# snarkify/sirius

Measured on AMD Instinct MI355X. Metric: IVC fold-steps/s (CycleFold IVC::next hot path, Poseidon-shaped synthetic trace, 2^k rows), higher is better.
Workload: dtype u256 (modular; 9 x 29-bit / 8 x 32-bit limbs)

## Files before the change

sirius_amd/csrc/msm.h:

```cpp
#pragma once
#include "curve.cuh"
#include "devrt.h"
#include "glv.cuh"
#include "stripes.h"
#include "tuning.h"

#include <cstdlib>

namespace srs {
namespace msm {

constexpr int WBITS = 16;
constexpr int NWIN = 16;
constexpr int NWIN_COMPACT = 8;
constexpr uint32_t PAY_ENDO = 1u << 30;
constexpr uint32_t NBUCKET = 1u << (WBITS - 1);

constexpr uint32_t SORT_THREADS = 1024;
constexpr uint32_t SORT_TILE_MIN = 8192;
constexpr uint32_t SORT_TARGET_BLOCKS = 256;
constexpr uint32_t SEG = 128, SEG_BUCKETS = NBUCKET / SEG;
constexpr uint32_t SORT_TILE2 = 8192;
constexpr uint64_t TWO_PASS_MIN_SLOTS = 1ull << 23;
constexpr uint32_t PLAN_THREADS = 1024;
constexpr uint32_t ACC_THREADS = 256;
constexpr uint32_t ACC_L0_LOG = 4, ACC_L0 = 1u << ACC_L0_LOG;
constexpr uint32_t ACC_L1_LOG = 3, ACC_L1 = 1u << ACC_L1_LOG;
constexpr uint32_t FINAL_THREADS = 256;
constexpr uint32_t FINAL_FANIN = 512;
constexpr int MAX_LEVELS = 8;
constexpr uint32_t RED_ROWS = 256;
constexpr uint32_t RED_COLS = NBUCKET / RED_ROWS;
constexpr uint32_t RED_THREADS = 4 * RED_COLS;
constexpr uint32_t ACC1_QUAD_MAX = 1u << 17;
constexpr uint32_t BATCH_ARGS = 16;
constexpr uint32_t LANDING_SLOTS = 16;
constexpr uint32_t NORM_G = 16;
constexpr uint32_t SLOT_LOG = 6;
constexpr uint32_t SLOT_L0_MIN_LOG = 2, SLOT_L0_MAX_LOG = 16;
constexpr int WBITS_W = 20;
constexpr int NWIN_W = 13;
constexpr uint32_t NSEG_W = 16;
// ... 63 lines not shown
```

sirius_amd/csrc/msm.hip:

```cpp
#define SRS_F29_CHAIN 1
#include "msm.h"
#include "tuning.h"
#include "curve29.cuh"
#include "prof.h"

#include <algorithm>
#include <cstdlib>
#include <numeric>
#include <vector>

namespace srs {
namespace msm {

__device__ __forceinline__ uint32_t upper_bucket(const uint32_t *__restrict__ tp, uint32_t t) {
    uint32_t lo = 0, hi = NBUCKET;
    while (hi - lo > 1) {
        uint32_t mid = (lo + hi) >> 1;
        if (tp[mid] <= t) lo = mid; else hi = mid;
    }
    return lo;
}

template <class C>
__global__ void k_table_step(const affine_t *__restrict__ prev, xyzz_t *__restrict__ tmp, uint32_t n, int nbits) {
// ... 88 lines not shown
    gen.x = F::one();
    if (C::ID == 0) {
        gen.y = F::dbl(F::one());
    } else {
        fe_t y;
        const uint32_t yc[8] = {0x823f272cu, 0x833fc48du, 0xf1181294u, 0x2d270d45u, 0x06a45d63u, 0xcf135e75u, 0x00000002u, 0u};
        for (int j = 0; j < 8; ++j) y.v[j] = yc[j];
        gen.y = F::to_mont(y);
    }
    tmp[i] = Ec<C>::mul_canon(k, gen);
}

template <class C>
__global__ void k_on_curve(const affine_t *__restrict__ pts, uint32_t n, uint32_t *__restrict__ bad) {
    uint32_t i = blockIdx.x * blockDim.x + threadIdx.x;
    if (i >= n) return;
    if (!Ec<C>::is_on_curve(table_unform<C>(pts[i]))) atomicAdd(bad, 1u);
}

struct BatchDesc {
    const fe_t *ptr[BATCH_ARGS];
    uint32_t n[BATCH_ARGS];
    uint32_t base[BATCH_ARGS];
};

__device__ __forceinline__ void recode_half(const uint32_t (&k)[4], bool neg, uint16_t *__restrict__ d, size_t n) {
    const uint32_t top = neg ? 0x7FFFu : 0x8000u;
    uint32_t carry = 0;
#pragma unroll
    for (int w = 0; w < NWIN_COMPACT; ++w) {
        const uint32_t v = ((k[w >> 1] >> ((w & 1) * 16)) & 0xFFFFu) + carry;
        const bool borrow = v > top;
        const uint32_t mag = borrow ? 0x10000u - v : v;
        const bool minus = borrow != neg;
        carry = borrow ? 1u : 0u;
        d[(size_t)w * n] = (uint16_t)(mag ? ((mag - 1u) | (minus ? 0x8000u : 0u)) : 0xFFFFu);
    }
}

template <class C, bool COMPACT>
__global__ void k_digits(BatchDesc bd, uint16_t *__restrict__ dig, size_t dig_stride, int is_mont, uint32_t rank, uint32_t world,
                         uint32_t *__restrict__ count_zero, uint32_t n_zero) {
    using S = typename C::S;
    uint32_t m = blockIdx.y;
    uint32_t n = bd.n[m];
    uint32_t i = blockIdx.x * blockDim.x + threadIdx.x;
    for (uint32_t j = (blockIdx.y * gridDim.x + blockIdx.x) * blockDim.x + threadIdx.x; j < n_zero; j += gridDim.x * gridDim.y * blockDim.x)
        count_zero[j] = 0;
    if (i >= n) return;
    fe_t s = bd.ptr[m][Stripes{rank, world}.global_index((size_t)i)];
    if (is_mont) s = S::from_mont(s);
    uint16_t *d = dig + (size_t)m * dig_stride;
    if (COMPACT) {
        const glv_t g = glv_decompose<C>(s);
        recode_half(g.k1, g.neg1, d + i, n);
        recode_half(g.k2, g.neg2, d + (size_t)NWIN_COMPACT * n + i, n);
        return;
    }
    uint32_t carry = 0;
#pragma unroll
    for (int w = 0; w < NWIN; ++w) {
        uint32_t raw = (s.v[w >> 1] >> ((w & 1) * 16)) & 0xFFFFu;
        uint32_t v = raw + carry;
        uint32_t code;
        if (v > 0x8000u) {
            code = ((0x10000u - v) - 1u) | 0x8000u;
            carry = 1;
        } else {
            code = v ? (v - 1u) : 0xFFFFu;
            carry = 0;
        }
        d[(size_t)w * n + i] = (uint16_t)code;
    }
}

template <class Fn>
__device__ __forceinline__ void for_each_digit(const uint16_t *__restrict__ d, uint32_t lo, uint32_t hi, Fn fn) {
    uint32_t head = lo;
    while (head < hi && (reinterpret_cast<uintptr_t>(d + head) & 15u)) ++head;
    for (uint32_t i = lo + threadIdx.x; i < head; i += blockDim.x) fn(i, (uint32_t)d[i]);
    const uint32_t nvec = (hi - head) / 8;
    const uint4 *v = reinterpret_cast<const uint4 *>(d + head);
    auto eight = [&](uint32_t q, const uint4 &x) {
        const uint32_t i0 = head + q * 8;
        fn(i0 + 0, x.x & 0xFFFFu); fn(i0 + 1, x.x >> 16);
        fn(i0 + 2, x.y & 0xFFFFu); fn(i0 + 3, x.y >> 16);
        fn(i0 + 4, x.z & 0xFFFFu); fn(i0 + 5, x.z >> 16);
        fn(i0 + 6, x.w & 0xFFFFu); fn(i0 + 7, x.w >> 16);
    };
    uint32_t q = threadIdx.x;
    for (; q + 3 * blockDim.x < nvec; q += 4 * blockDim.x) {
        const uint4 x0 = v[q], x1 = v[q + blockDim.x], x2 = v[q + 2 * blockDim.x], x3 = v[q + 3 * blockDim.x];
        eight(q, x0); eight(q + blockDim.x, x1); eight(q + 2 * blockDim.x, x2); eight(q + 3 * blockDim.x, x3);
    }
    for (; q < nvec; q += blockDim.x) eight(q, v[q]);
    for (uint32_t i = head + nvec * 8 + threadIdx.x; i < hi; i += blockDim.x) fn(i, (uint32_t)d[i]);
}

__device__ __forceinline__ void tile_histogram(uint32_t *h, const uint16_t *__restrict__ d, uint32_t lo, uint32_t hi) {
    for (uint32_t b = threadIdx.x; b < NBUCKET; b += blockDim.x) h[b] = 0;
    __syncthreads();
    for_each_digit(d, lo, hi, [&](uint32_t, uint32_t code) {
        if (code != 0xFFFFu) atomicAdd(&h[code & 0x7FFFu], 1u);
    });
    __syncthreads();
}

__global__ void SRS_KERNEL_BOUNDS(SORT_THREADS, 1)
    k_hist(const uint16_t *__restrict__ dig, size_t dig_stride, BatchDesc bd,
           uint32_t *__restrict__ count , uint32_t SORT_TILE,
           uint32_t *__restrict__ tile_hist ) {
    __shared__ uint32_t h[NBUCKET];
    uint32_t m = blockIdx.z, w = blockIdx.y;
    uint32_t n = bd.n[m];
    uint32_t lo = blockIdx.x * SORT_TILE;
    const uint32_t T1 = gridDim.x * NWIN, t1 = w * gridDim.x + blockIdx.x;
    if (lo >= n) {
        if (tile_hist)
            for (uint32_t sgm = threadIdx.x; sgm < SEG; sgm += blockDim.x) tile_hist[((size_t)m * SEG + sgm) * T1 + t1] = 0;
        return;
    }
    uint32_t hi = lo + SORT_TILE < n ? lo + SORT_TILE : n;
    const uint16_t *d = dig + (size_t)m * dig_stride + (size_t)w * n;
    tile_histogram(h, d, lo, hi);
    uint32_t *cnt = count + (size_t)m * NBUCKET;
    const uint32_t rot = ((blockIdx.y * gridDim.x + blockIdx.x) * 128u) & (NBUCKET - 1);
    for (uint32_t i = threadIdx.x; i < NBUCKET; i += blockDim.x) {
        const uint32_t b = (i + rot) & (NBUCKET - 1);
        uint32_t c = h[b];
        if (c) atomicAdd(&cnt[b], c);
    }
    if (tile_hist) {
        for (uint32_t sgm = threadIdx.x; sgm < SEG; sgm += blockDim.x) {
            uint32_t c = 0;
            for (uint32_t b = 0; b < SEG_BUCKETS; ++b) c += h[sgm * SEG_BUCKETS + ((b + sgm) & (SEG_BUCKETS - 1))];
            tile_hist[((size_t)m * SEG + sgm) * T1 + t1] = c;
        }
    }
}

__device__ __forceinline__ uint32_t block_exclusive_scan(uint32_t v, uint32_t *lds, uint32_t *total);

__global__ void SRS_KERNEL_BOUNDS(1024, 1)
    k_scan_seg(uint32_t *__restrict__ tile_hist, uint32_t T1, const uint32_t *__restrict__ plan, size_t plan_stride) {
    __shared__ uint32_t lds[64];
    const uint32_t sgm = blockIdx.x, m = blockIdx.y;
    uint32_t *row = tile_hist + ((size_t)m * SEG + sgm) * T1;
    const uint32_t base = plan[(size_t)m * plan_stride + (size_t)sgm * SEG_BUCKETS];
    uint32_t carry = 0;
    for (uint32_t at = 0; at < T1; at += blockDim.x) {
        const uint32_t i = at + threadIdx.x;
        const uint32_t v = i < T1 ? row[i] : 0;
        uint32_t total;
        const uint32_t ex = block_exclusive_scan(v, lds, &total);
        if (i < T1) row[i] = base + carry + ex;
        carry += total;
    }
}

constexpr uint32_t GRP_PER = 16, GRP_SUB = SORT_THREADS * GRP_PER;
template <bool COMPACT>
__device__ __forceinline__ uint32_t payload_base(uint32_t w, uint32_t table_stride, uint32_t base) {
    if (COMPACT) return ((w & (NWIN_COMPACT - 1)) * table_stride + base) | (w >= NWIN_COMPACT ? PAY_ENDO : 0u);
    return w * table_stride + base;
}
template <bool COMPACT>
__global__ void SRS_KERNEL_BOUNDS(SORT_THREADS, 1)
    k_group(const uint16_t *__restrict__ dig, size_t dig_stride, BatchDesc bd, const uint32_t *__restrict__ tile_hist,
            uint16_t *__restrict__ gkey, uint32_t *__restrict__ gpay, size_t g_stride, uint32_t table_stride, uint32_t SORT_TILE,
            const uint32_t *__restrict__ plan, size_t plan_stride, uint16_t *__restrict__ tb, size_t tb_stride, uint32_t arr) {
    __shared__ uint32_t cur[SEG], cnt[SEG], lb[SEG], sc[64];
    __shared__ uint32_t spay[GRP_SUB];
    __shared__ uint16_t skey[GRP_SUB];
    const uint32_t m = blockIdx.z, w = blockIdx.y, tid = threadIdx.x;
    if (tb) {
        const uint32_t *tp = plan + (size_t)m * plan_stride + (size_t)arr * (NBUCKET + 1);
        uint16_t *map = tb + (size_t)m * tb_stride;
        const uint32_t waves = gridDim.x * gridDim.y * (blockDim.x >> 6);
        const uint32_t wv = (blockIdx.y * gridDim.x + blockIdx.x) * (blockDim.x >> 6) + (tid >> 6), lane = tid & 63u;
        for (uint32_t b = wv; b < NBUCKET; b += waves) {
            const uint32_t s = tp[b], e = tp[b + 1];
            for (uint32_t t = s + lane; t < e; t += 64) map[t] = (uint16_t)b;
        }
    }
    const uint32_t n = bd.n[m];
    const uint32_t lo = blockIdx.x * SORT_TILE;
    if (lo >= n) return;
    const uint32_t hi = lo + SORT_TILE < n ? lo + SORT_TILE : n;
    const uint32_t T1 = gridDim.x * NWIN, t1 = w * gridDim.x + blockIdx.x;
    for (uint32_t sgm = tid; sgm < SEG; sgm += blockDim.x) cur[sgm] = tile_hist[((size_t)m * SEG + sgm) * T1 + t1];
    const uint16_t *d = dig + (size_t)m * dig_stride + (size_t)w * n;
    uint16_t *ok = gkey + (size_t)m * g_stride;
    uint32_t *op = gpay + (size_t)m * g_stride;
    const uint32_t pay0 = payload_base<COMPACT>(w, table_stride, bd.base[m]);
    for (uint32_t sub = lo; sub < hi; sub += GRP_SUB) {
        for (uint32_t sgm = tid; sgm < SEG; sgm += blockDim.x) cnt[sgm] = 0;
        __syncthreads();
        const uint32_t i0 = sub + tid * GRP_PER;
        uint32_t code[GRP_PER], rank[GRP_PER];
        if (i0 + GRP_PER <= hi && (reinterpret_cast<uintptr_t>(d + i0) & 15u) == 0) {
            const uint4 *v = reinterpret_cast<const uint4 *>(d + i0);
#pragma unroll
            for (uint32_t q = 0; q < GRP_PER / 8; ++q) {
                const uint4 x = v[q];
                code[8 * q + 0] = x.x & 0xFFFFu; code[8 * q + 1] = x.x >> 16;
                code[8 * q + 2] = x.y & 0xFFFFu; code[8 * q + 3] = x.y >> 16;
                code[8 * q + 4] = x.z & 0xFFFFu; code[8 * q + 5] = x.z >> 16;
                code[8 * q + 6] = x.w & 0xFFFFu; code[8 * q + 7] = x.w >> 16;
            }
        } else {
#pragma unroll
            for (uint32_t k = 0; k < GRP_PER; ++k) code[k] = i0 + k < hi ? (uint32_t)d[i0 + k] : 0xFFFFu;
        }
#pragma unroll
        for (uint32_t k = 0; k < GRP_PER; ++k)
            rank[k] = code[k] != 0xFFFFu ? atomicAdd(&cnt[(code[k] & 0x7FFFu) / SEG_BUCKETS], 1u) : 0u;
        __syncthreads();
        uint32_t n_sub;
        const uint32_t ex = block_exclusive_scan(tid < SEG ? cnt[tid] : 0u, sc, &n_sub);
        if (tid < SEG) lb[tid] = ex;
        __syncthreads();
#pragma unroll
        for (uint32_t k = 0; k < GRP_PER; ++k) {
            if (code[k] != 0xFFFFu) {
                const uint32_t bkt = code[k] & 0x7FFFu, pos = lb[bkt / SEG_BUCKETS] + rank[k];
                skey[pos] = (uint16_t)bkt;
                spay[pos] = (pay0 + i0 + k) | ((code[k] & 0x8000u) << 16);
            }
        }
        __syncthreads();
        for (uint32_t i = tid; i < n_sub; i += blockDim.x) {
            const uint32_t key = skey[i], sgm = key / SEG_BUCKETS, g = cur[sgm] + (i - lb[sgm]);
            ok[g] = (uint16_t)key;
            op[g] = spay[i];
        }
        __syncthreads();
        if (tid < SEG) cur[tid] += cnt[tid];
    }
}

constexpr uint32_t S2_PER = 8, S2_RANGE = 2 * SEG_BUCKETS;
static_assert(SORT_TILE2 == SORT_THREADS * S2_PER, "k_scatter2: one tile = S2_PER entries per thread");
__global__ void SRS_KERNEL_BOUNDS(SORT_THREADS, 2)
    k_scatter2(const uint16_t *__restrict__ gkey, const uint32_t *__restrict__ gpay, size_t g_stride,
               const uint32_t *__restrict__ plan, size_t plan_stride, uint32_t *__restrict__ cursor ,
               uint32_t *__restrict__ sorted, size_t sorted_stride, uint32_t TILE2) {
    __shared__ uint32_t cnt[S2_RANGE], lb[S2_RANGE], gb[S2_RANGE], sc[64];
    __shared__ uint32_t spay[SORT_TILE2];
    __shared__ uint16_t skey[SORT_TILE2];
    const uint32_t m = blockIdx.y, tid = threadIdx.x;
    const uint32_t total = plan[(size_t)m * plan_stride + NBUCKET];
    const uint32_t n_tiles = (total + TILE2 - 1) / TILE2, per_xcd = (n_tiles + 7) / 8;
    if (blockIdx.x / 8 >= per_xcd) return;
    const uint32_t tile_id = (blockIdx.x % 8) * per_xcd + blockIdx.x / 8;
    if (tile_id >= n_tiles) return;
    const uint32_t lo = tile_id * TILE2;
    if (lo >= total) return;
    const uint32_t hi = lo + TILE2 < total ? lo + TILE2 : total;
    const uint16_t *key = gkey + (size_t)m * g_stride;
    const uint32_t *pay = gpay + (size_t)m * g_stride;
// ... 31 lines not shown
    if (tid < S2_RANGE) {
        lb[tid] = ex;
        gb[tid] = c ? atomicAdd(&cur[b_lo + tid], c) : 0u;
    }
    __syncthreads();
#pragma unroll
    for (uint32_t k = 0; k < S2_PER; ++k) {
        if (kk[k] != 0xFFFFu) {
            const uint32_t pos = lb[kk[k] - b_lo] + rank[k];
            skey[pos] = (uint16_t)(kk[k] - b_lo);
            spay[pos] = pp[k];
        }
    }
    __syncthreads();
    for (uint32_t i = tid; i < n_tile; i += blockDim.x) {
        const uint32_t b = skey[i];
        out[gb[b] + (i - lb[b])] = spay[i];
    }
}

#ifndef SCATTER_RES_INFLIGHT
#define SCATTER_RES_INFLIGHT 4
#endif
template <bool COMPACT>
__global__ void SRS_KERNEL_BOUNDS(SORT_THREADS, 1)
    k_scatter(const uint16_t *__restrict__ dig, size_t dig_stride, BatchDesc bd,
              uint32_t *__restrict__ cursor , uint32_t *__restrict__ sorted,
              size_t sorted_stride, uint32_t table_stride, uint32_t SORT_TILE) {
    __shared__ uint32_t h[NBUCKET];
    uint32_t m = blockIdx.z, w = blockIdx.y;
    uint32_t n = bd.n[m];
    uint32_t lo = blockIdx.x * SORT_TILE;
    if (lo >= n) return;
    uint32_t hi = lo + SORT_TILE < n ? lo + SORT_TILE : n;
    const uint16_t *d = dig + (size_t)m * dig_stride + (size_t)w * n;
    tile_histogram(h, d, lo, hi);
    uint32_t *cur = cursor + (size_t)m * NBUCKET;
    constexpr int RES = SCATTER_RES_INFLIGHT;
    for (uint32_t b0 = threadIdx.x; b0 < NBUCKET; b0 += RES * blockDim.x) {
        uint32_t c[RES], r[RES];
#pragma unroll
        for (int u = 0; u < RES; ++u) c[u] = b0 + u * blockDim.x < NBUCKET ? h[b0 + u * blockDim.x] : 0u;
#pragma unroll
        for (int u = 0; u < RES; ++u) r[u] = c[u] ? atomicAdd(&cur[b0 + u * blockDim.x], c[u]) : 0u;
#pragma unroll
        for (int u = 0; u < RES; ++u) if (c[u]) h[b0 + u * blockDim.x] = r[u];
    }
    __syncthreads();
    uint32_t *out = sorted + (size_t)m * sorted_stride;
    const uint32_t pay0 = payload_base<COMPACT>(w, table_stride, bd.base[m]);
    for_each_digit(d, lo, hi, [&](uint32_t i, uint32_t code) {
        if (code != 0xFFFFu) {
            uint32_t pos = atomicAdd(&h[code & 0x7FFFu], 1u);
            out[pos] = (pay0 + i) | ((code & 0x8000u) << 16);
        }
    });
}

struct Link {
    uint32_t base[MAX_LEVELS + 1][NSEG_W + 1];
};
__device__ __forceinline__ uint32_t link_segment(const uint32_t *__restrict__ base, uint32_t t) {
    uint32_t v = 0;
#pragma unroll
    for (uint32_t u = 1; u < NSEG_W; ++u) v += (t >= base[u]) ? 1u : 0u;
    return v;
}

struct WideDesc {
    const fe_t *ptr;
    uint32_t n, base;
    uint32_t rank, world;
    int is_mont;
};

template <class C>
__device__ __forceinline__ void wide_codes(const WideDesc &wd, uint32_t i, uint32_t (&code)[NWIN_W]) {
// ... 1159 lines not shown
    return (lg >= 2 && lg <= 8) ? (uint32_t)lg : SLOT_LOG;
}
static uint32_t slot_want_cap() { return 4u; }

struct LevelShape {
    uint64_t M;
    int levels;
    size_t plan_stride;
    uint64_t cap0, cap1;
    uint32_t quad_max;
};
struct SetShape : LevelShape {
    bool two_pass;
    uint32_t tile, tiles;
};
struct NarrowShape : SetShape { uint32_t l0_log; };
struct SlotShape : SetShape { uint32_t S, nred; };
struct WideShape : LevelShape { uint32_t l0_log, T, tiles_g; };

static void sort_shape(SetShape &h, uint32_t n_max, uint32_t batch) {
    h.M = (uint64_t)n_max * NWIN;
    h.quad_max = acc1_quad_max();
    h.two_pass = use_two_pass(h.M, batch);
    h.tile = (uint32_t)((h.M * batch + SORT_TARGET_BLOCKS - 1) / SORT_TARGET_BLOCKS);
    h.tile = (h.tile + 1023u) & ~1023u;
    if (h.tile < SORT_TILE_MIN) h.tile = SORT_TILE_MIN;
    h.tiles = ceil_div(n_max, h.tile);
}
static NarrowShape narrow_shape(uint32_t n_max, uint32_t batch) {
    NarrowShape h;
    sort_shape(h, n_max, batch);
    h.l0_log = l0_log_for(h.M);
    h.levels = levels_for((h.M + (1ull << h.l0_log) - 1) >> h.l0_log);
    h.plan_stride = (size_t)(h.levels + 1) * (NBUCKET + 1) + 4;
    h.cap0 = (h.M >> h.l0_log) + NBUCKET + 1;
    h.cap1 = h.cap0 / ACC_L1 + NBUCKET + 1;
    return h;
}
static SlotShape slot_shape(uint32_t n_max, uint32_t batch) {
    SlotShape h;
    sort_shape(h, n_max, batch);
    const uint32_t lg = slot_log();
    h.S = 1u << lg;
    h.nred = (lg + 2) / 3;
    h.cap0 = std::min<uint64_t>((uint64_t)NBUCKET * h.S, (h.M >> SLOT_L0_MIN_LOG) + NBUCKET);
    h.cap1 = h.cap0 / ACC_L1 + NBUCKET + 1;
    h.levels = levels_for(h.cap0);
    h.plan_stride = (size_t)(h.levels + 2) * (NBUCKET + 1) + 4;
// ... 22 lines not shown
    }
};
template <class Walk>
static size_t sized(Walk walk) {
    Sizer s;
    walk(s);
    return s.used;
}
template <class Walk>
static auto carve(Arena &A, Walk walk) {
    const size_t need = sized(walk);
    A.reserve(need);
    A.reset();
    const auto bufs = walk(A);
    if (A.used != need) {
        set_error("internal: msm workspace: the arena walk and the sizer disagree");
        throw DeviceError{5};
    }
    return bufs;
}

struct SetBufs {
    xyzz_t *d_out, *ping, *pong, *rc;
    uint16_t *dig, *tb;
    uint32_t *sorted, *count, *cursor, *plan;
    uint16_t *gkey;
    uint32_t *gpay, *tile_hist;
};
struct NarrowBufs : SetBufs { xyzz_t *buckets; };
struct SlotBufs : SetBufs { xyzz_t *red_a, *red_b; };
template <class W>
static void take_set_head(W &A, const SetShape &h, uint32_t batch, SetBufs &b) {
    b.d_out = A.template take<xyzz_t>(3 * (size_t)batch);
    b.dig = A.template take<uint16_t>(h.M * batch);
    b.sorted = A.template take<uint32_t>(h.M * batch);
    b.count = A.template take<uint32_t>((size_t)NBUCKET * batch);
    b.cursor = A.template take<uint32_t>((size_t)NBUCKET * batch);
    b.plan = A.template take<uint32_t>(h.plan_stride * batch);
    b.ping = A.template take<xyzz_t>(h.cap0 * batch);
    b.tb = A.template take<uint16_t>(h.cap0 * batch);
    b.pong = A.template take<xyzz_t>(h.cap1 * batch);
}
template <class W>
static void take_set_tail(W &A, const SetShape &h, uint32_t batch, SetBufs &b) {
    b.rc = A.template take<xyzz_t>((size_t)(RED_ROWS + RED_COLS) * batch);
    b.gkey = h.two_pass ? A.template take<uint16_t>(h.M * batch) : nullptr;
    b.gpay = h.two_pass ? A.template take<uint32_t>(h.M * batch) : nullptr;
    b.tile_hist = h.two_pass ? A.template take<uint32_t>((size_t)SEG * (SORT_TARGET_BLOCKS + 2 * NWIN) * batch) : nullptr;
}
template <class W>
static NarrowBufs narrow_layout(W &A, const NarrowShape &h, uint32_t batch) {
    NarrowBufs b;
    take_set_head(A, h, batch, b);
    b.buckets = A.template take<xyzz_t>((size_t)NBUCKET * batch);
    take_set_tail(A, h, batch, b);
    return b;
}
template <class W>
static SlotBufs slot_layout(W &A, const SlotShape &h, uint32_t batch) {
    SlotBufs b;
    take_set_head(A, h, batch, b);
    b.red_a = A.template take<xyzz_t>((size_t)NBUCKET * (h.S / 8 + 1) * batch);
    b.red_b = A.template take<xyzz_t>((size_t)NBUCKET * (h.S / 64 + 1) * batch);
    take_set_tail(A, h, batch, b);
    return b;
}
struct WideBufs {
    xyzz_t *d_out, *d_seg, *ping, *pong, *buckets, *rc;
    uint16_t *gkey, *gkey2, *tb;
    uint32_t *gpay, *gpay2, *tile_cnt, *tile_hist;
    uint32_t *seg3;
// ... 17 lines not shown
    b.count = A.template take<uint32_t>((size_t)NSEG_W * NBUCKET);
    b.cursor = A.template take<uint32_t>((size_t)NSEG_W * NBUCKET);
    b.plan = A.template take<uint32_t>(w.plan_stride * NSEG_W);
    b.ping = A.template take<xyzz_t>(w.cap0);
    b.tb = A.template take<uint16_t>(w.cap0);
    b.pong = A.template take<xyzz_t>(w.cap1);
    b.buckets = A.template take<xyzz_t>((size_t)NSEG_W * NBUCKET);
    b.rc = A.template take<xyzz_t>((size_t)NSEG_W * (RED_ROWS + RED_COLS));
    return b;
}

size_t workspace_bytes(uint32_t n_max, uint32_t batch) {
    return sized([&](auto &A) { return narrow_layout(A, narrow_shape(n_max, batch), batch); });
}
static size_t workspace_bytes_slots(uint32_t n_max, uint32_t batch) {
    return sized([&](auto &A) { return slot_layout(A, slot_shape(n_max, batch), batch); });
}
static size_t workspace_bytes_wide(uint32_t n) {
    return sized([&](auto &A) { return wide_layout(A, wide_shape(n)); });
}

template <class C, class LaunchPlan>
static void sort_front(const Key &k, const SetShape &h, const SetBufs &b, const fe_t *const *scalars_dev, const uint32_t *n_host,
                       const uint32_t *base_host, uint32_t batch, uint32_t n_max, int is_mont, hipStream_t stream, LaunchPlan launch_plan,
                       bool group_maps, uint32_t arr) {
    BatchDesc bd;
    for (uint32_t m = 0; m < BATCH_ARGS; ++m) {
        bd.ptr[m] = m < batch ? scalars_dev[m] : nullptr;
        bd.n[m] = m < batch ? n_host[m] : 0;
        bd.base[m] = (m < batch && base_host) ? base_host[m] : 0;
    }
    const uint32_t s_rank = k.compact_scalars ? 0u : k.rank, s_world = k.compact_scalars ? 1u : k.world;
    const size_t M = (size_t)h.M;
    const auto digits = k.compact ? &k_digits<C, true> : &k_digits<C, false>;
    const auto group = k.compact ? &k_group<true> : &k_group<false>;
    const auto scatter = k.compact ? &k_scatter<true> : &k_scatter<false>;
    SRS_LAUNCH(digits, (ceil_div(n_max, 256), batch), (256), 0, stream, bd, b.dig, M, is_mont, s_rank, s_world, b.count,
               (uint32_t)(NBUCKET * batch));
    SRS_LAUNCH(k_hist, (h.tiles, NWIN, batch), (SORT_THREADS), 0, stream, (const uint16_t *)b.dig, M, bd, b.count, h.tile, b.tile_hist);
    launch_plan();
    if (h.two_pass) {
        const uint32_t T1 = h.tiles * NWIN;
        SRS_LAUNCH(k_scan_seg, (SEG, batch), (1024), 0, stream, b.tile_hist, T1, (const uint32_t *)b.plan, h.plan_stride);
        SRS_LAUNCH(group, (h.tiles, NWIN, batch), (SORT_THREADS), 0, stream, (const uint16_t *)b.dig, M, bd, (const uint32_t *)b.tile_hist,
                   b.gkey, b.gpay, M, (uint32_t)k.len, h.tile, group_maps ? (const uint32_t *)b.plan : nullptr,
                   group_maps ? h.plan_stride : (size_t)0, group_maps ? b.tb : nullptr, group_maps ? (size_t)h.cap0 : (size_t)0,
                   group_maps ? arr : 0u);
        SRS_LAUNCH(k_scatter2, (8 * ceil_div(ceil_div(M, SORT_TILE2), 8), batch), (SORT_THREADS), 0, stream, (const uint16_t *)b.gkey,
                   (const uint32_t *)b.gpay, M, (const uint32_t *)b.plan, h.plan_stride, b.cursor, b.sorted, M, (uint32_t)SORT_TILE2);
    } else {
        SRS_LAUNCH(scatter, (h.tiles, NWIN, batch), (SORT_THREADS), 0, stream, (const uint16_t *)b.dig, M, bd, b.cursor, b.sorted, M,
                   (uint32_t)k.len, h.tile);
    }
    if (!(h.two_pass && group_maps))
        SRS_LAUNCH(k_expand, (NBUCKET / 4, batch), (256), 0, stream, (const uint32_t *)b.plan, h.plan_stride, b.tb, (size_t)h.cap0,
                   (const Link *)nullptr, arr);
}

struct Parts {
    const uint32_t *plan; size_t plan_stride;
    xyzz_t *ping; size_t stride0;
    xyzz_t *pong; size_t stride1;
    const Link *link;
};

template <class C>
static void accum_levels(const Parts &p, const LevelShape &h, uint64_t cap_inc, uint32_t batch, hipStream_t stream) {
    xyzz_t *cur = p.ping, *nxt = p.pong;
    size_t cur_stride = p.stride0, nxt_stride = p.stride1;
    uint64_t cap = h.cap0;
    for (int level = 1; level < h.levels; ++level) {
        cap = cap / ACC_L1 + cap_inc;
        SRS_LAUNCH((k_accum1<C>), (ceil_div(std::max<uint64_t>(cap, 4 * std::min<uint64_t>(cap, h.quad_max)), ACC_THREADS), batch),
                   (ACC_THREADS), 0, stream, (const xyzz_t *)cur, cur_stride, p.plan, h.plan_stride, level, nxt, nxt_stride, (uint32_t)ACC_L1,
                   p.link, h.quad_max);
// ... 2 lines not shown
    }
}

template <class C>
static void reduce_buckets(const Parts &p, uint32_t nmsm, const xyzz_t *from, int from_buckets, xyzz_t *rc, uint32_t sums, xyzz_t *d_sums,
                           hipStream_t stream) {
    SRS_LAUNCH((k_rowcol<C>), (RED_ROWS / 2 + RED_COLS, nmsm), (128), 0, stream, from, (const xyzz_t *)p.ping, p.stride0,
               (const xyzz_t *)p.pong, p.stride1, p.plan, p.plan_stride, rc, p.link, from_buckets);
    SRS_LAUNCH((k_reduce_final<C>), (sums, nmsm), (RED_THREADS), 0, stream, (const xyzz_t *)rc, d_sums);
}

static void land(Key &k, const xyzz_t *d_out, size_t n, uint32_t slot, hipStream_t stream) {
    if (!k.h_result) SRS_HIP_CHECK(hipHostMalloc(&k.h_result, 3 * (size_t)BATCH_ARGS * LANDING_SLOTS * sizeof(xyzz_t)));
    xyzz_t *dst = static_cast<xyzz_t *>(k.h_result) + 3 * (size_t)BATCH_ARGS * slot;
    SRS_HIP_CHECK(hipMemcpyAsync(dst, d_out, n * sizeof(xyzz_t), hipMemcpyDeviceToHost, stream));
}

template <class C>
static bool enqueue_t(Key &k, const fe_t *const *scalars_dev, const uint32_t *n_host, const uint32_t *base_host, uint32_t batch,
                      uint32_t n_max, int is_mont, hipStream_t stream, uint32_t slot, Fold fold) {
    if (n_max == 0) return false;
    const NarrowShape h = narrow_shape(n_max, batch);
    const NarrowBufs b = carve(k.arena, [&](auto &A) { return narrow_layout(A, h, batch); });
    sort_front<C>(k, h, b, scalars_dev, n_host, base_host, batch, n_max, is_mont, stream, [&] {
        SRS_LAUNCH(k_plan, (batch, h.levels + 1), (PLAN_THREADS), 0, stream, (const uint32_t *)b.count, b.cursor, b.plan, h.plan_stride,
                   h.levels, h.l0_log, (uint32_t)ACC_L1_LOG, (const uint32_t *)nullptr);
    }, false, 1u);
    const Parts p{b.plan, h.plan_stride, b.ping, (size_t)h.cap0, b.pong, (size_t)h.cap1, nullptr};
    const uint64_t units = std::accumulate(n_host, n_host + batch, (uint64_t)0);
    const auto accum0 = k.compact ? &k_accum0c<C> : &k_accum0<C>;
    SRS_LAUNCH_TIMED("msm_accum0", units, accum0, (ceil_div(h.cap0, ACC_THREADS), batch), (ACC_THREADS), 0, stream,
                     (const uint32_t *)b.sorted, (size_t)h.M, p.plan, p.plan_stride, (const uint16_t *)b.tb, p.stride0,
                     (const affine_t *)k.table, p.ping, p.stride0, 1u << h.l0_log, p.link);
    accum_levels<C>(p, h, NBUCKET + 1, batch, stream);
    SRS_LAUNCH((k_accum_final<C>), (NBUCKET / (FINAL_THREADS / 64), batch), (FINAL_THREADS), 0, stream, (const xyzz_t *)p.ping, p.stride0,
               (const xyzz_t *)p.pong, p.stride1, p.plan, p.plan_stride, b.buckets, p.link);
    const xyzz_t *red_from = b.buckets;
    int from_buckets = 0;
    if (fold != FOLD_NONE) {
        if (!k.fold_buckets) SRS_HIP_CHECK(hipMalloc((void **)&k.fold_buckets, (size_t)NBUCKET * sizeof(xyzz_t)));
        SRS_LAUNCH((k_bucket_fold<C>), (NBUCKET / 64), (64), 0, stream, (const xyzz_t *)b.buckets, (const xyzz_t *)p.ping,
                   (const xyzz_t *)p.pong, p.plan, p.plan_stride, k.fold_buckets, fold == FOLD_FIRST ? 1 : 0);
        if (fold != FOLD_LAST) return true;
        red_from = k.fold_buckets;
        from_buckets = 1;
    }
    reduce_buckets<C>(p, batch, red_from, from_buckets, b.rc, 3, b.d_out, stream);
// ... 24 lines not shown
        const size_t need = (size_t)batch * NBUCKET * S;
        if (k.slots_pts < need) {
            if (k.slots) SRS_HIP_CHECK(hipFree(k.slots));
            k.slots = nullptr;
            k.slots_pts = 0;
            SRS_HIP_CHECK(hipMalloc((void **)&k.slots, need * sizeof(xyzz_t)));
            k.slots_pts = need;
        }
        if (!k.used) SRS_HIP_CHECK(hipMalloc((void **)&k.used, 2 * (size_t)BATCH_ARGS * NBUCKET));
        if (!k.h_ovf) {
            SRS_HIP_CHECK(hipHostMalloc((void **)&k.h_ovf, 2 * (size_t)LANDING_SLOTS * BATCH_ARGS * sizeof(uint32_t)));
            for (size_t i = 0; i < 2 * (size_t)LANDING_SLOTS * BATCH_ARGS; ++i) k.h_ovf[i] = 0;
        }
    } else if (k.slot_s != S || batch != 1) {
        set_error("internal: msm slot mode: a commit's sets must share the slot layout");
        throw DeviceError{5};
    }
    const uint8_t *used_prev = k.used + (size_t)(k.seq & 1u) * BATCH_ARGS * NBUCKET;
    uint8_t *used_next = k.used + (size_t)((k.seq + 1) & 1u) * BATCH_ARGS * NBUCKET;
    ++k.seq;

    const SlotBufs b = carve(k.arena, [&](auto &A) { return slot_layout(A, h, batch); });
    const uint32_t arr = (uint32_t)h.levels + 1;
    sort_front<C>(k, h, b, scalars_dev, n_host, base_host, batch, n_max, is_mont, stream, [&] {
        SRS_LAUNCH(k_plan_s, (batch, h.levels + 2), (PLAN_THREADS), 0, stream, (const uint32_t *)b.count, b.cursor, b.plan, h.plan_stride,
                   h.levels, S, (uint32_t)ACC_L1_LOG, used_prev, used_next, first ? 1 : 0, k.h_ovf + (size_t)slot * BATCH_ARGS, slot_want_cap());
    }, true, arr);
    const Parts p{b.plan, h.plan_stride, b.ping, (size_t)h.cap0, b.pong, (size_t)h.cap1, nullptr};
    const uint64_t units = std::accumulate(n_host, n_host + batch, (uint64_t)0);
    const auto accum0s = k.compact ? &k_accum0sc<C> : &k_accum0s<C>;
    SRS_LAUNCH_TIMED("msm_accum0", units, accum0s, (ceil_div(h.cap0, ACC_THREADS), batch), (ACC_THREADS), 0, stream,
                     (const uint32_t *)b.sorted, (size_t)h.M, p.plan, p.plan_stride, arr, (const uint16_t *)b.tb, p.stride0,
                     (const affine_t *)k.table, k.slots, S, used_prev, first ? 1 : 0, p.ping, p.stride0);
    if (k.commit_ovf) {
        accum_levels<C>(p, h, NBUCKET + 1, batch, stream);
        SRS_LAUNCH((k_ovf_final<C>), (NBUCKET / (FINAL_THREADS / 64), batch), (FINAL_THREADS), 0, stream, (const xyzz_t *)p.ping, p.stride0,
                   (const xyzz_t *)p.pong, p.stride1, p.plan, p.plan_stride, k.slots, S, first ? 1 : 0);
    }
    k.landing[slot] = {false, true, k.commit_ovf, batch};
    ++k.stat_slot_sets;
    if (!last) return true;
    const xyzz_t *in = k.slots;
    uint32_t in_pb = S;
    xyzz_t *outs[2] = {b.red_a, b.red_b};
    for (uint32_t l = 0; l < h.nred; ++l) {
        const uint32_t out_pb = (in_pb + 7) / 8, n_out = NBUCKET * out_pb;
        xyzz_t *out = outs[l & 1u];
// ... 220 lines not shown
```

Before: 99.93.

## Fuse scalar digit recoding into MSM histogram, group and scatter kernels

Drops the separate digit-recoding kernel and its 16-bit digit buffer. The histogram, group and scatter kernels now load scalars directly and recompute the signed window codes in registers for all windows per scalar. Tiling changes from per-window to per-scalar, with a smaller minimum tile and a wave-shuffle reduction for the per-segment tile histogram. This saves a kernel launch and the digit buffer's global write and reads, but repeats Montgomery conversion and GLV decomposition in each sort kernel and raises register pressure.

```diff
diff --git a/sirius_amd/csrc/msm.h b/sirius_amd/csrc/msm.h
--- a/sirius_amd/csrc/msm.h
+++ b/sirius_amd/csrc/msm.h
@@ -17,7 +17,7 @@
 constexpr uint32_t NBUCKET = 1u << (WBITS - 1);
 
 constexpr uint32_t SORT_THREADS = 1024;
-constexpr uint32_t SORT_TILE_MIN = 8192;
+constexpr uint32_t SORT_TILE_MIN = 512;
 constexpr uint32_t SORT_TARGET_BLOCKS = 256;
 constexpr uint32_t SEG = 128, SEG_BUCKETS = NBUCKET / SEG;
 constexpr uint32_t SORT_TILE2 = 8192;
diff --git a/sirius_amd/csrc/msm.hip b/sirius_amd/csrc/msm.hip
--- a/sirius_amd/csrc/msm.hip
+++ b/sirius_amd/csrc/msm.hip
@@ -134,9 +134,12 @@
     const fe_t *ptr[BATCH_ARGS];
     uint32_t n[BATCH_ARGS];
     uint32_t base[BATCH_ARGS];
+    uint32_t rank, world;
+    int is_mont;
 };
 
-__device__ __forceinline__ void recode_half(const uint32_t (&k)[4], bool neg, uint16_t *__restrict__ d, size_t n) {
+template <int W0>
+__device__ __forceinline__ void recode_half(const uint32_t (&k)[4], bool neg, uint32_t (&code)[NWIN]) {
     const uint32_t top = neg ? 0x7FFFu : 0x8000u;
     uint32_t carry = 0;
 #pragma unroll
@@ -146,45 +149,45 @@
         const uint32_t mag = borrow ? 0x10000u - v : v;
         const bool minus = borrow != neg;
         carry = borrow ? 1u : 0u;
-        d[(size_t)w * n] = (uint16_t)(mag ? ((mag - 1u) | (minus ? 0x8000u : 0u)) : 0xFFFFu);
+        code[W0 + w] = mag ? ((mag - 1u) | (minus ? 0x8000u : 0u)) : 0xFFFFu;
     }
 }
 
 template <class C, bool COMPACT>
-__global__ void k_digits(BatchDesc bd, uint16_t *__restrict__ dig, size_t dig_stride, int is_mont, uint32_t rank, uint32_t world,
-                         uint32_t *__restrict__ count_zero, uint32_t n_zero) {
-    using S = typename C::S;
-    uint32_t m = blockIdx.y;
-    uint32_t n = bd.n[m];
-    uint32_t i = blockIdx.x * blockDim.x + threadIdx.x;
-    for (uint32_t j = (blockIdx.y * gridDim.x + blockIdx.x) * blockDim.x + threadIdx.x; j < n_zero; j += gridDim.x * gridDim.y * blockDim.x)
-        count_zero[j] = 0;
-    if (i >= n) return;
-    fe_t s = bd.ptr[m][Stripes{rank, world}.global_index((size_t)i)];
-    if (is_mont) s = S::from_mont(s);
-    uint16_t *d = dig + (size_t)m * dig_stride;
-    if (COMPACT) {
-        const glv_t g = glv_decompose<C>(s);
-        recode_half(g.k1, g.neg1, d + i, n);
-        recode_half(g.k2, g.neg2, d + (size_t)NWIN_COMPACT * n + i, n);
-        return;
-    }
-    uint32_t carry = 0;
-#pragma unroll
-    for (int w = 0; w < NWIN; ++w) {
-        uint32_t raw = (s.v[w >> 1] >> ((w & 1) * 16)) & 0xFFFFu;
-        uint32_t v = raw + carry;
-        uint32_t code;
-        if (v > 0x8000u) {
-            code = ((0x10000u - v) - 1u) | 0x8000u;
-            carry = 1;
-        } else {
-            code = v ? (v - 1u) : 0xFFFFu;
-            carry = 0;
-        }
-        d[(size_t)w * n + i] = (uint16_t)code;
-    }
-}
+struct ScalarCodes {
+    const fe_t *ptr;
+    Stripes st;
+    int is_mont;
+    __device__ __forceinline__ ScalarCodes(const BatchDesc &bd, uint32_t m) : ptr(bd.ptr[m]), st{bd.rank, bd.world}, is_mont(bd.is_mont) {}
+    __device__ __forceinline__ fe_t load(uint32_t i) const { return ptr[st.global_index((size_t)i)]; }
+    __device__ __forceinline__ void codes(fe_t s, uint32_t (&code)[NWIN]) const {
+        using S = typename C::S;
+        if ((s.v[0] | s.v[1] | s.v[2] | s.v[3] | s.v[4] | s.v[5] | s.v[6] | s.v[7]) == 0) {
+#pragma unroll
+            for (int w = 0; w < NWIN; ++w) code[w] = 0xFFFFu;
+            return;
+        }
+        if (is_mont) s = S::from_mont(s);
+        if (COMPACT) {
+            const glv_t g = glv_decompose<C>(s);
+            recode_half<0>(g.k1, g.neg1, code);
+            recode_half<NWIN_COMPACT>(g.k2, g.neg2, code);
+            return;
+        }
+        uint32_t carry = 0;
+#pragma unroll
+        for (int w = 0; w < NWIN; ++w) {
+            const uint32_t v = ((s.v[w >> 1] >> ((w & 1) * 16)) & 0xFFFFu) + carry;
+            if (v > 0x8000u) {
+                code[w] = (((0x10000u - v) - 1u) | 0x8000u) & 0xFFFFu;
+                carry = 1;
+            } else {
+                code[w] = v ? (v - 1u) : 0xFFFFu;
+                carry = 0;
+            }
+        }
+    }
+};
 
 template <class Fn>
 __device__ __forceinline__ void for_each_digit(const uint16_t *__restrict__ d, uint32_t lo, uint32_t hi, Fn fn) {
@@ -218,36 +221,69 @@
     __syncthreads();
 }
 
+constexpr uint32_t SCALARS_INFLIGHT = 4;
+template <class C, bool COMPACT, class Fn>
+__device__ __forceinline__ void for_each_scalar(const ScalarCodes<C, COMPACT> &sc, uint32_t lo, uint32_t hi, Fn fn) {
+    static_assert(SCALARS_INFLIGHT == 4, "for_each_scalar: the register queue below holds four scalars");
+    for (uint32_t i0 = lo + threadIdx.x; i0 < hi; i0 += SCALARS_INFLIGHT * blockDim.x) {
+        fe_t s0 = sc.load(i0), s1 = fe_t{}, s2 = fe_t{}, s3 = fe_t{};
+        if (i0 + blockDim.x < hi) s1 = sc.load(i0 + blockDim.x);
+        if (i0 + 2 * blockDim.x < hi) s2 = sc.load(i0 + 2 * blockDim.x);
+        if (i0 + 3 * blockDim.x < hi) s3 = sc.load(i0 + 3 * blockDim.x);
+#pragma unroll 1
+        for (uint32_t i = i0; i < hi && i < i0 + SCALARS_INFLIGHT * blockDim.x; i += blockDim.x) {
+            uint32_t code[NWIN];
+            sc.codes(s0, code);
+            fn(i, code);
+            s0 = s1; s1 = s2; s2 = s3;
+        }
+    }
+}
+
+template <class C, bool COMPACT>
+__device__ __forceinline__ void tile_histogram_s(uint32_t *h, const ScalarCodes<C, COMPACT> &sc, uint32_t lo, uint32_t hi) {
+    for (uint32_t b = threadIdx.x; b < NBUCKET; b += blockDim.x) h[b] = 0;
+    __syncthreads();
+    for_each_scalar(sc, lo, hi, [&](uint32_t, const uint32_t (&code)[NWIN]) {
+#pragma unroll
+        for (int w = 0; w < NWIN; ++w)
+            if (code[w] != 0xFFFFu) atomicAdd(&h[code[w] & 0x7FFFu], 1u);
+    });
+    __syncthreads();
+}
+
+template <class C, bool COMPACT>
 __global__ void SRS_KERNEL_BOUNDS(SORT_THREADS, 1)
-    k_hist(const uint16_t *__restrict__ dig, size_t dig_stride, BatchDesc bd,
-           uint32_t *__restrict__ count , uint32_t SORT_TILE,
+    k_hist(BatchDesc bd, uint32_t *__restrict__ count , uint32_t SORT_TILE,
            uint32_t *__restrict__ tile_hist ) {
     __shared__ uint32_t h[NBUCKET];
-    uint32_t m = blockIdx.z, w = blockIdx.y;
-    uint32_t n = bd.n[m];
-    uint32_t lo = blockIdx.x * SORT_TILE;
-    const uint32_t T1 = gridDim.x * NWIN, t1 = w * gridDim.x + blockIdx.x;
+    const uint32_t m = blockIdx.y;
+    const uint32_t n = bd.n[m];
+    const uint32_t lo = blockIdx.x * SORT_TILE;
+    const uint32_t T1 = gridDim.x, t1 = blockIdx.x;
     if (lo >= n) {
         if (tile_hist)
             for (uint32_t sgm = threadIdx.x; sgm < SEG; sgm += blockDim.x) tile_hist[((size_t)m * SEG + sgm) * T1 + t1] = 0;
         return;
     }
-    uint32_t hi = lo + SORT_TILE < n ? lo + SORT_TILE : n;
-    const uint16_t *d = dig + (size_t)m * dig_stride + (size_t)w * n;
-    tile_histogram(h, d, lo, hi);
+    const uint32_t hi = SORT_TILE < n - lo ? lo + SORT_TILE : n;
+    tile_histogram_s(h, ScalarCodes<C, COMPACT>(bd, m), lo, hi);
     uint32_t *cnt = count + (size_t)m * NBUCKET;
-    const uint32_t rot = ((blockIdx.y * gridDim.x + blockIdx.x) * 128u) & (NBUCKET - 1);
+    const uint32_t rot = (blockIdx.x * 128u) & (NBUCKET - 1);
     for (uint32_t i = threadIdx.x; i < NBUCKET; i += blockDim.x) {
         const uint32_t b = (i + rot) & (NBUCKET - 1);
         uint32_t c = h[b];
         if (c) atomicAdd(&cnt[b], c);
     }
     if (tile_hist) {
-        for (uint32_t sgm = threadIdx.x; sgm < SEG; sgm += blockDim.x) {
-            uint32_t c = 0;
-            for (uint32_t b = 0; b < SEG_BUCKETS; ++b) c += h[sgm * SEG_BUCKETS + ((b + sgm) & (SEG_BUCKETS - 1))];
-            tile_hist[((size_t)m * SEG + sgm) * T1 + t1] = c;
-        }
+        static_assert(SORT_THREADS == SEG * 8 && SEG_BUCKETS == 256, "k_hist: 8 lanes x 32 counters per segment");
+        const uint32_t sgm = threadIdx.x >> 3, l = threadIdx.x & 7u;
+        uint32_t c = 0;
+        for (uint32_t j = 0; j < SEG_BUCKETS / 8; ++j) c += h[sgm * SEG_BUCKETS + ((l + 8u * (j + sgm)) & (SEG_BUCKETS - 1))];
+        c += __shfl_xor(c, 1, 64);
+        c += __shfl_xor(c, 2, 64);
+        c += __shfl_xor(c, 4, 64);
+        if (l == 0) tile_hist[((size_t)m * SEG + sgm) * T1 + t1] = c;
     }
 }
 
@@ -270,26 +306,26 @@
     }
 }
 
-constexpr uint32_t GRP_PER = 16, GRP_SUB = SORT_THREADS * GRP_PER;
+constexpr uint32_t GRP_PER = NWIN, GRP_SUB = SORT_THREADS * GRP_PER;
 template <bool COMPACT>
 __device__ __forceinline__ uint32_t payload_base(uint32_t w, uint32_t table_stride, uint32_t base) {
     if (COMPACT) return ((w & (NWIN_COMPACT - 1)) * table_stride + base) | (w >= NWIN_COMPACT ? PAY_ENDO : 0u);
     return w * table_stride + base;
 }
-template <bool COMPACT>
+template <class C, bool COMPACT>
 __global__ void SRS_KERNEL_BOUNDS(SORT_THREADS, 1)
-    k_group(const uint16_t *__restrict__ dig, size_t dig_stride, BatchDesc bd, const uint32_t *__restrict__ tile_hist,
+    k_group(BatchDesc bd, const uint32_t *__restrict__ tile_hist,
             uint16_t *__restrict__ gkey, uint32_t *__restrict__ gpay, size_t g_stride, uint32_t table_stride, uint32_t SORT_TILE,
             const uint32_t *__restrict__ plan, size_t plan_stride, uint16_t *__restrict__ tb, size_t tb_stride, uint32_t arr) {
     __shared__ uint32_t cur[SEG], cnt[SEG], lb[SEG], sc[64];
     __shared__ uint32_t spay[GRP_SUB];
     __shared__ uint16_t skey[GRP_SUB];
-    const uint32_t m = blockIdx.z, w = blockIdx.y, tid = threadIdx.x;
+    const uint32_t m = blockIdx.y, tid = threadIdx.x;
     if (tb) {
         const uint32_t *tp = plan + (size_t)m * plan_stride + (size_t)arr * (NBUCKET + 1);
         uint16_t *map = tb + (size_t)m * tb_stride;
-        const uint32_t waves = gridDim.x * gridDim.y * (blockDim.x >> 6);
-        const uint32_t wv = (blockIdx.y * gridDim.x + blockIdx.x) * (blockDim.x >> 6) + (tid >> 6), lane = tid & 63u;
+        const uint32_t waves = gridDim.x * (blockDim.x >> 6);
+        const uint32_t wv = blockIdx.x * (blockDim.x >> 6) + (tid >> 6), lane = tid & 63u;
         for (uint32_t b = wv; b < NBUCKET; b += waves) {
             const uint32_t s = tp[b], e = tp[b + 1];
             for (uint32_t t = s + lane; t < e; t += 64) map[t] = (uint16_t)b;
@@ -298,32 +334,21 @@
     const uint32_t n = bd.n[m];
     const uint32_t lo = blockIdx.x * SORT_TILE;
     if (lo >= n) return;
-    const uint32_t hi = lo + SORT_TILE < n ? lo + SORT_TILE : n;
-    const uint32_t T1 = gridDim.x * NWIN, t1 = w * gridDim.x + blockIdx.x;
+    const uint32_t hi = SORT_TILE < n - lo ? lo + SORT_TILE : n;
+    const uint32_t T1 = gridDim.x, t1 = blockIdx.x;
     for (uint32_t sgm = tid; sgm < SEG; sgm += blockDim.x) cur[sgm] = tile_hist[((size_t)m * SEG + sgm) * T1 + t1];
-    const uint16_t *d = dig + (size_t)m * dig_stride + (size_t)w * n;
+    const ScalarCodes<C, COMPACT> src(bd, m);
     uint16_t *ok = gkey + (size_t)m * g_stride;
     uint32_t *op = gpay + (size_t)m * g_stride;
-    const uint32_t pay0 = payload_base<COMPACT>(w, table_stride, bd.base[m]);
-    for (uint32_t sub = lo; sub < hi; sub += GRP_SUB) {
+    const uint32_t base = bd.base[m];
+    fe_t s = lo + tid < hi ? src.load(lo + tid) : fe_t{};
+    for (uint32_t sub = lo; sub < hi; sub += SORT_THREADS) {
         for (uint32_t sgm = tid; sgm < SEG; sgm += blockDim.x) cnt[sgm] = 0;
         __syncthreads();
-        const uint32_t i0 = sub + tid * GRP_PER;
+        const uint32_t i = sub + tid;
+        const fe_t nxt = i + SORT_THREADS < hi ? src.load(i + SORT_THREADS) : fe_t{};
         uint32_t code[GRP_PER], rank[GRP_PER];
-        if (i0 + GRP_PER <= hi && (reinterpret_cast<uintptr_t>(d + i0) & 15u) == 0) {
-            const uint4 *v = reinterpret_cast<const uint4 *>(d + i0);
-#pragma unroll
-            for (uint32_t q = 0; q < GRP_PER / 8; ++q) {
-                const uint4 x = v[q];
-                code[8 * q + 0] = x.x & 0xFFFFu; code[8 * q + 1] = x.x >> 16;
-                code[8 * q + 2] = x.y & 0xFFFFu; code[8 * q + 3] = x.y >> 16;
-                code[8 * q + 4] = x.z & 0xFFFFu; code[8 * q + 5] = x.z >> 16;
-                code[8 * q + 6] = x.w & 0xFFFFu; code[8 * q + 7] = x.w >> 16;
-            }
-        } else {
-#pragma unroll
-            for (uint32_t k = 0; k < GRP_PER; ++k) code[k] = i0 + k < hi ? (uint32_t)d[i0 + k] : 0xFFFFu;
-        }
+        src.codes(s, code);
 #pragma unroll
         for (uint32_t k = 0; k < GRP_PER; ++k)
             rank[k] = code[k] != 0xFFFFu ? atomicAdd(&cnt[(code[k] & 0x7FFFu) / SEG_BUCKETS], 1u) : 0u;
@@ -337,17 +362,18 @@
             if (code[k] != 0xFFFFu) {
                 const uint32_t bkt = code[k] & 0x7FFFu, pos = lb[bkt / SEG_BUCKETS] + rank[k];
                 skey[pos] = (uint16_t)bkt;
-                spay[pos] = (pay0 + i0 + k) | ((code[k] & 0x8000u) << 16);
+                spay[pos] = (payload_base<COMPACT>(k, table_stride, base) + i) | ((code[k] & 0x8000u) << 16);
             }
         }
         __syncthreads();
-        for (uint32_t i = tid; i < n_sub; i += blockDim.x) {
-            const uint32_t key = skey[i], sgm = key / SEG_BUCKETS, g = cur[sgm] + (i - lb[sgm]);
+        for (uint32_t j = tid; j < n_sub; j += blockDim.x) {
+            const uint32_t key = skey[j], sgm = key / SEG_BUCKETS, g = cur[sgm] + (j - lb[sgm]);
             ok[g] = (uint16_t)key;
-            op[g] = spay[i];
+            op[g] = spay[j];
         }
         __syncthreads();
         if (tid < SEG) cur[tid] += cnt[tid];
+        s = nxt;
     }
 }
 
@@ -425,19 +451,18 @@
 #ifndef SCATTER_RES_INFLIGHT
 #define SCATTER_RES_INFLIGHT 4
 #endif
-template <bool COMPACT>
+template <class C, bool COMPACT>
 __global__ void SRS_KERNEL_BOUNDS(SORT_THREADS, 1)
-    k_scatter(const uint16_t *__restrict__ dig, size_t dig_stride, BatchDesc bd,
-              uint32_t *__restrict__ cursor , uint32_t *__restrict__ sorted,
+    k_scatter(BatchDesc bd, uint32_t *__restrict__ cursor , uint32_t *__restrict__ sorted,
               size_t sorted_stride, uint32_t table_stride, uint32_t SORT_TILE) {
     __shared__ uint32_t h[NBUCKET];
-    uint32_t m = blockIdx.z, w = blockIdx.y;
-    uint32_t n = bd.n[m];
-    uint32_t lo = blockIdx.x * SORT_TILE;
+    const uint32_t m = blockIdx.y;
+    const uint32_t n = bd.n[m];
+    const uint32_t lo = blockIdx.x * SORT_TILE;
     if (lo >= n) return;
-    uint32_t hi = lo + SORT_TILE < n ? lo + SORT_TILE : n;
-    const uint16_t *d = dig + (size_t)m * dig_stride + (size_t)w * n;
-    tile_histogram(h, d, lo, hi);
+    const uint32_t hi = SORT_TILE < n - lo ? lo + SORT_TILE : n;
+    const ScalarCodes<C, COMPACT> src(bd, m);
+    tile_histogram_s(h, src, lo, hi);
     uint32_t *cur = cursor + (size_t)m * NBUCKET;
     constexpr int RES = SCATTER_RES_INFLIGHT;
     for (uint32_t b0 = threadIdx.x; b0 < NBUCKET; b0 += RES * blockDim.x) {
@@ -451,11 +476,14 @@
     }
     __syncthreads();
     uint32_t *out = sorted + (size_t)m * sorted_stride;
-    const uint32_t pay0 = payload_base<COMPACT>(w, table_stride, bd.base[m]);
-    for_each_digit(d, lo, hi, [&](uint32_t i, uint32_t code) {
-        if (code != 0xFFFFu) {
-            uint32_t pos = atomicAdd(&h[code & 0x7FFFu], 1u);
-            out[pos] = (pay0 + i) | ((code & 0x8000u) << 16);
+    const uint32_t base = bd.base[m];
+    for_each_scalar(src, lo, hi, [&](uint32_t i, const uint32_t (&code)[NWIN]) {
+#pragma unroll
+        for (uint32_t w = 0; w < NWIN; ++w) {
+            if (code[w] != 0xFFFFu) {
+                const uint32_t pos = atomicAdd(&h[code[w] & 0x7FFFu], 1u);
+                out[pos] = (payload_base<COMPACT>(w, table_stride, base) + i) | ((code[w] & 0x8000u) << 16);
+            }
         }
     });
 }
@@ -1661,8 +1689,8 @@
     h.M = (uint64_t)n_max * NWIN;
     h.quad_max = acc1_quad_max();
     h.two_pass = use_two_pass(h.M, batch);
-    h.tile = (uint32_t)((h.M * batch + SORT_TARGET_BLOCKS - 1) / SORT_TARGET_BLOCKS);
-    h.tile = (h.tile + 1023u) & ~1023u;
+    h.tile = (uint32_t)(((uint64_t)n_max * batch + SORT_TARGET_BLOCKS - 1) / SORT_TARGET_BLOCKS);
+    h.tile = (h.tile + 63u) & ~63u;
     if (h.tile < SORT_TILE_MIN) h.tile = SORT_TILE_MIN;
     h.tiles = ceil_div(n_max, h.tile);
 }
@@ -1731,7 +1759,7 @@
 
 struct SetBufs {
     xyzz_t *d_out, *ping, *pong, *rc;
-    uint16_t *dig, *tb;
+    uint16_t *tb;
     uint32_t *sorted, *count, *cursor, *plan;
     uint16_t *gkey;
     uint32_t *gpay, *tile_hist;
@@ -1741,7 +1769,6 @@
 template <class W>
 static void take_set_head(W &A, const SetShape &h, uint32_t batch, SetBufs &b) {
     b.d_out = A.template take<xyzz_t>(3 * (size_t)batch);
-    b.dig = A.template take<uint16_t>(h.M * batch);
     b.sorted = A.template take<uint32_t>(h.M * batch);
     b.count = A.template take<uint32_t>((size_t)NBUCKET * batch);
     b.cursor = A.template take<uint32_t>((size_t)NBUCKET * batch);
@@ -1755,7 +1782,7 @@
     b.rc = A.template take<xyzz_t>((size_t)(RED_ROWS + RED_COLS) * batch);
     b.gkey = h.two_pass ? A.template take<uint16_t>(h.M * batch) : nullptr;
     b.gpay = h.two_pass ? A.template take<uint32_t>(h.M * batch) : nullptr;
-    b.tile_hist = h.two_pass ? A.template take<uint32_t>((size_t)SEG * (SORT_TARGET_BLOCKS + 2 * NWIN) * batch) : nullptr;
+    b.tile_hist = h.two_pass ? A.template take<uint32_t>((size_t)SEG * (SORT_TARGET_BLOCKS + 1) * batch) : nullptr;
 }
 template <class W>
 static NarrowBufs narrow_layout(W &A, const NarrowShape &h, uint32_t batch) {
@@ -1819,7 +1846,7 @@
 
 template <class C, class LaunchPlan>
 static void sort_front(const Key &k, const SetShape &h, const SetBufs &b, const fe_t *const *scalars_dev, const uint32_t *n_host,
-                       const uint32_t *base_host, uint32_t batch, uint32_t n_max, int is_mont, hipStream_t stream, LaunchPlan launch_plan,
+                       const uint32_t *base_host, uint32_t batch, int is_mont, hipStream_t stream, LaunchPlan launch_plan,
                        bool group_maps, uint32_t arr) {
     BatchDesc bd;
     for (uint32_t m = 0; m < BATCH_ARGS; ++m) {
@@ -1827,27 +1854,26 @@
         bd.n[m] = m < batch ? n_host[m] : 0;
         bd.base[m] = (m < batch && base_host) ? base_host[m] : 0;
     }
-    const uint32_t s_rank = k.compact_scalars ? 0u : k.rank, s_world = k.compact_scalars ? 1u : k.world;
+    bd.rank = k.compact_scalars ? 0u : k.rank;
+    bd.world = k.compact_scalars ? 1u : k.world;
+    bd.is_mont = is_mont;
     const size_t M = (size_t)h.M;
-    const auto digits = k.compact ? &k_digits<C, true> : &k_digits<C, false>;
-    const auto group = k.compact ? &k_group<true> : &k_group<false>;
-    const auto scatter = k.compact ? &k_scatter<true> : &k_scatter<false>;
-    SRS_LAUNCH(digits, (ceil_div(n_max, 256), batch), (256), 0, stream, bd, b.dig, M, is_mont, s_rank, s_world, b.count,
-               (uint32_t)(NBUCKET * batch));
-    SRS_LAUNCH(k_hist, (h.tiles, NWIN, batch), (SORT_THREADS), 0, stream, (const uint16_t *)b.dig, M, bd, b.count, h.tile, b.tile_hist);
+    const auto hist = k.compact ? &k_hist<C, true> : &k_hist<C, false>;
+    const auto group = k.compact ? &k_group<C, true> : &k_group<C, false>;
+    const auto scatter = k.compact ? &k_scatter<C, true> : &k_scatter<C, false>;
+    SRS_HIP_CHECK(hipMemsetAsync(b.count, 0, (size_t)NBUCKET * batch * sizeof(uint32_t), stream));
+    SRS_LAUNCH(hist, (h.tiles, batch), (SORT_THREADS), 0, stream, bd, b.count, h.tile, b.tile_hist);
     launch_plan();
     if (h.two_pass) {
-        const uint32_t T1 = h.tiles * NWIN;
-        SRS_LAUNCH(k_scan_seg, (SEG, batch), (1024), 0, stream, b.tile_hist, T1, (const uint32_t *)b.plan, h.plan_stride);
-        SRS_LAUNCH(group, (h.tiles, NWIN, batch), (SORT_THREADS), 0, stream, (const uint16_t *)b.dig, M, bd, (const uint32_t *)b.tile_hist,
+        SRS_LAUNCH(k_scan_seg, (SEG, batch), (1024), 0, stream, b.tile_hist, h.tiles, (const uint32_t *)b.plan, h.plan_stride);
+        SRS_LAUNCH(group, (h.tiles, batch), (SORT_THREADS), 0, stream, bd, (const uint32_t *)b.tile_hist,
                    b.gkey, b.gpay, M, (uint32_t)k.len, h.tile, group_maps ? (const uint32_t *)b.plan : nullptr,
                    group_maps ? h.plan_stride : (size_t)0, group_maps ? b.tb : nullptr, group_maps ? (size_t)h.cap0 : (size_t)0,
                    group_maps ? arr : 0u);
         SRS_LAUNCH(k_scatter2, (8 * ceil_div(ceil_div(M, SORT_TILE2), 8), batch), (SORT_THREADS), 0, stream, (const uint16_t *)b.gkey,
                    (const uint32_t *)b.gpay, M, (const uint32_t *)b.plan, h.plan_stride, b.cursor, b.sorted, M, (uint32_t)SORT_TILE2);
     } else {
-        SRS_LAUNCH(scatter, (h.tiles, NWIN, batch), (SORT_THREADS), 0, stream, (const uint16_t *)b.dig, M, bd, b.cursor, b.sorted, M,
-                   (uint32_t)k.len, h.tile);
+        SRS_LAUNCH(scatter, (h.tiles, batch), (SORT_THREADS), 0, stream, bd, b.cursor, b.sorted, M, (uint32_t)k.len, h.tile);
     }
     if (!(h.two_pass && group_maps))
         SRS_LAUNCH(k_expand, (NBUCKET / 4, batch), (256), 0, stream, (const uint32_t *)b.plan, h.plan_stride, b.tb, (size_t)h.cap0,
@@ -1896,7 +1922,7 @@
     if (n_max == 0) return false;
     const NarrowShape h = narrow_shape(n_max, batch);
     const NarrowBufs b = carve(k.arena, [&](auto &A) { return narrow_layout(A, h, batch); });
-    sort_front<C>(k, h, b, scalars_dev, n_host, base_host, batch, n_max, is_mont, stream, [&] {
+    sort_front<C>(k, h, b, scalars_dev, n_host, base_host, batch, is_mont, stream, [&] {
         SRS_LAUNCH(k_plan, (batch, h.levels + 1), (PLAN_THREADS), 0, stream, (const uint32_t *)b.count, b.cursor, b.plan, h.plan_stride,
                    h.levels, h.l0_log, (uint32_t)ACC_L1_LOG, (const uint32_t *)nullptr);
     }, false, 1u);
@@ -1967,7 +1993,7 @@
 
     const SlotBufs b = carve(k.arena, [&](auto &A) { return slot_layout(A, h, batch); });
     const uint32_t arr = (uint32_t)h.levels + 1;
-    sort_front<C>(k, h, b, scalars_dev, n_host, base_host, batch, n_max, is_mont, stream, [&] {
+    sort_front<C>(k, h, b, scalars_dev, n_host, base_host, batch, is_mont, stream, [&] {
         SRS_LAUNCH(k_plan_s, (batch, h.levels + 2), (PLAN_THREADS), 0, stream, (const uint32_t *)b.count, b.cursor, b.plan, h.plan_stride,
                    h.levels, S, (uint32_t)ACC_L1_LOG, used_prev, used_next, first ? 1 : 0, k.h_ovf + (size_t)slot * BATCH_ARGS, slot_want_cap());
     }, true, arr);
```

Result: no change. 99.27 (-0.7%).
